# L-Scofano/SEEME

Measured on AMD Instinct MI355X. Metric: sampled seqs/sec (T=196, 50 DDIM steps), higher is better.
Workload: dtype f32 accumulate (fp16 denoiser weights, fp16 VAE MFMA operands); 1 GPU; config_mld_egobody interactee-only: VAE encode -> 50-step DDIM -> VAE decode, B=32/GPU, T=196, nfeats=132, random-init recipe weights; batch_per_gpu=32, seq_len=196, ddim_steps=50, parallelism=dp1 (independent shards, no collective on the data path)

## Files before the change

include/seeme_hip.h:

```cpp
#ifndef SEEME_HIP_H
#define SEEME_HIP_H

#include <stddef.h>
#include <stdint.h>

#ifdef __cplusplus
extern "C" {
#endif

#define SEEME_D 256
#define SEEME_NLAYERS 5

enum { SEEME_ACT_NONE = 0, SEEME_ACT_RELU = 1, SEEME_ACT_GELU = 2, SEEME_ACT_SILU = 3 };
enum { SEEME_SCHED_NONE = 0, SEEME_SCHED_DDIM = 1, SEEME_SCHED_DDPM = 2 };

int seeme_version(void);
const char* seeme_last_error(void);

#define SEEME_LINEAR_MAX_K 1008
typedef struct {
    const float* A;  int lda;
    const float* A2; int lda2;
    int K1;
    const float* W;  int ldw;
// ... 11 lines not shown

typedef struct {
    const float *in_w, *in_b;
    const float *out_w, *out_b;
    const float *l1_w, *l1_b;
    const float *l2_w, *l2_b;
    const float *n1_w, *n1_b, *n2_w, *n2_b;
    const float *ca_in_w, *ca_in_b;
    const float *ca_out_w, *ca_out_b;
    const float *n3_w, *n3_b;
} SeemeXfLayer;

typedef struct {
    SeemeXfLayer layer[SEEME_NLAYERS];
    const float *skip_w[2], *skip_b[2];
    const float *norm_w, *norm_b;
} SeemeSkipStack;

typedef struct { const uint16_t *in_w, *out_w, *l1_w, *l2_w; } SeemeXfLayerH;
typedef struct {
    SeemeXfLayerH enc[SEEME_NLAYERS], dec[SEEME_NLAYERS];
    const uint16_t *enc_skip[2], *dec_skip[2];
    const uint16_t *emb_w, *fin_w, *ca_fold_w;
    const void* dec_pro; int dec_pro_T;
} SeemeVaeWeightsH;

typedef struct {
    int nfeats;
    int ff;
    const float* token;
    const float* pe_enc;
    const float* pe_dec;
    const float* emb_w; int emb_ldw;
    const float* emb_b;
    const float* fin_w;
    const float* fin_b;
    SeemeSkipStack enc, dec;
    const float* ca_fold_w;
    const float* ca_fold_b;
    const SeemeVaeWeightsH* h16;
} SeemeVaeWeights;

size_t seeme_vae_workspace_bytes(int B, int T);

int seeme_vae_encode(const SeemeVaeWeights* w, const float* features, const int32_t* lengths,
                     int B, int T, float* mu, float* logvar, void* workspace, size_t ws_bytes, void* stream);

// ... 430 lines not shown
```

seeme_amd/_lib.py:

```python
from __future__ import annotations

import ctypes as C
import os
from typing import Optional

_HERE = os.path.dirname(os.path.abspath(__file__))
LIB_PATH = os.environ.get("SEEME_HIP_LIB") or os.path.join(_HERE, "libseeme_hip.so")

NLAYERS = 5
TROW = 7680
CROW = 5120
ACT_NONE, ACT_RELU, ACT_GELU, ACT_SILU = 0, 1, 2, 3
SCHED_NONE, SCHED_DDIM, SCHED_DDPM = 0, 1, 2

fp = C.c_void_p


class SeemeError(RuntimeError):
    pass


class LinearArgs(C.Structure):
    _fields_ = [("A", fp), ("lda", C.c_int), ("A2", fp), ("lda2", C.c_int), ("K1", C.c_int),
                ("W", fp), ("ldw", C.c_int), ("bias", fp), ("res", fp), ("ldr", C.c_int),
                ("ln_w", fp), ("ln_b", fp), ("pre_ln_w", fp), ("pre_ln_b", fp),
                ("Y", fp), ("ldy", C.c_int), ("M", C.c_int), ("N", C.c_int), ("K", C.c_int),
                ("pre_act", C.c_int), ("act", C.c_int), ("eps", C.c_float)]


class XfLayer(C.Structure):
    _fields_ = [(n, fp) for n in ("in_w", "in_b", "out_w", "out_b", "l1_w", "l1_b", "l2_w", "l2_b",
                                  "n1_w", "n1_b", "n2_w", "n2_b",
                                  "ca_in_w", "ca_in_b", "ca_out_w", "ca_out_b", "n3_w", "n3_b")]


class SkipStack(C.Structure):
    _fields_ = [("layer", XfLayer * NLAYERS), ("skip_w", fp * 2), ("skip_b", fp * 2),
                ("norm_w", fp), ("norm_b", fp)]


class XfLayerH(C.Structure):
    _fields_ = [(n, fp) for n in ("in_w", "out_w", "l1_w", "l2_w")]


class VaeWeightsH(C.Structure):
    _fields_ = [("enc", XfLayerH * NLAYERS), ("dec", XfLayerH * NLAYERS), ("enc_skip", fp * 2), ("dec_skip", fp * 2),
                ("emb_w", fp), ("fin_w", fp), ("ca_fold_w", fp), ("dec_pro", fp), ("dec_pro_T", C.c_int)]


def pack_mfma16(W, dtype):
    import torch
    N, K = W.shape
    Np, Kp = (N + 15) // 16 * 16, (K + 31) // 32 * 32
    Wz = torch.zeros(Np, Kp, device=W.device, dtype=dtype)
    Wz[:N, :K] = W.detach().to(dtype)
    return Wz.view(Np // 16, 16, Kp // 32, 4, 8).permute(0, 2, 3, 1, 4).contiguous()


class VaeWeights(C.Structure):
    _fields_ = [("nfeats", C.c_int), ("ff", C.c_int), ("token", fp), ("pe_enc", fp), ("pe_dec", fp),
                ("emb_w", fp), ("emb_ldw", C.c_int), ("emb_b", fp), ("fin_w", fp), ("fin_b", fp),
                ("enc", SkipStack), ("dec", SkipStack), ("ca_fold_w", fp), ("ca_fold_b", fp), ("h16", fp)]


class DenoiserWeights(C.Structure):
    _fields_ = [("wg", fp), ("wdtype", C.c_int), ("vp", fp), ("layout", fp), ("nhead", C.c_int), ("ff_sa", C.c_int),
                ("ff", C.c_int), ("kv_cat_w", fp), ("kv_cat_b", fp), ("style_cat_w", fp), ("style_cat_b", fp),
                ("time_w1", fp), ("time_b1", fp), ("time_w2", fp), ("time_b2", fp),
                ("ca_kv_w", fp * NLAYERS), ("ca_kv_b", fp * NLAYERS),
                ("ca_tn_w", fp * NLAYERS), ("ca_tn_b", fp * NLAYERS),
# ... 285 lines not shown
```

seeme_amd/csrc/vae_h16.hip:

```cpp
#include "common.hpp"
#include "api_util.hpp"

typedef _Float16 h16x8 __attribute__((ext_vector_type(8)));
#define HPAD 16

__device__ __forceinline__ unsigned short f2h(float x) { return __builtin_bit_cast(unsigned short, (_Float16)x); }
__device__ __forceinline__ float h_exp(float x) { return __builtin_amdgcn_exp2f(x * 1.44269504088896340736f); }
__device__ __forceinline__ float h_gelu(float x) {
    const float z = fabsf(x) * 0.70710678118654752440f;
    const float t = __builtin_amdgcn_rcpf(fmaf(0.3275911f, z, 1.f));
    const float poly = t * fmaf(t, fmaf(t, fmaf(t, fmaf(t, 1.061405429f, -1.453152027f), 1.421413741f), -0.284496736f), 0.254829592f);
    return 0.5f * x * (1.f + copysignf(1.f - poly * h_exp(-z * z), x));
}
__device__ __forceinline__ float h_act(float v, int act) { return act == SEEME_ACT_GELU ? h_gelu(v) : act_apply(v, act); }

#ifdef H16_DBG_TIMES
__device__ unsigned long long h16_dbg_times[32];
#ifndef H16_DBG_KERNEL
#define H16_DBG_KERNEL 1
#endif
#define H16_DBG(k, i) do { if (H16_DBG_KERNEL == (k) && blockIdx.x == 3 && blockIdx.y == ((k) == 1 ? 5 : 0) && threadIdx.x == 0) h16_dbg_times[i] = __builtin_readcyclecounter(); } while (0)
extern "C" int seeme_debug_h16_times(unsigned long long* host, int n) {
    SEEME_HIP(hipMemcpyFromSymbol(host, HIP_SYMBOL(h16_dbg_times), sizeof(unsigned long long) * (size_t)(n < 32 ? n : 32)));
    return 0;
// ... 691 lines not shown
#ifndef LAYER_KV_PF
#define LAYER_KV_PF 4
#endif
#ifndef LAYER_W8_PF
#define LAYER_W8_PF 4
#endif
#ifndef LAYER_WPE
#define LAYER_WPE 2
#endif
struct LayerHArgs {
    const unsigned short* q; const uint4* kp; const uint4* vp; const float* res;
    const uint4* wo; const float* bo; const float* n1_w; const float* n1_b;
    const int32_t* lengths;
    int S, n_prefix, q_rows, Sp, spv; float scale, eps;
    const float* cvec; int cvec_ld; const float* lnc_w; const float* lnc_b;
    const uint4* w1; const float* b1; const uint4* w2; const float* b2; const float* n2_w; const float* n2_b;
    const float* fin_w; const float* fin_b;
    float* out; int out_mode, B;
    int in_shared;
    const uint4* skip_w; const float* skip_b; const float* skip_src; float* xnext;
    const uint4* qkv_w; const float* qkv_b; unsigned short* q_out; uint4* kp_out; uint4* vp_out;
    const uint4* proj_w; const float* proj_b; float* feats; int F;
    const float* z; const uint4* cf_w; const float* cf_b; int layer;
};
template <int WAVES, int RW>
__host__ __device__ constexpr bool layer_cvec_in() { return WAVES == 8 && RW == 4; }

__device__ __forceinline__ void rows_to_h16(unsigned short* Xh, int ldh, int row, int lane, float4 v) {
    const unsigned lo = (unsigned)f2h(v.x) | ((unsigned)f2h(v.y) << 16), hi = (unsigned)f2h(v.z) | ((unsigned)f2h(v.w) << 16);
    *reinterpret_cast<uint2*>(Xh + row * ldh + lane * 4) = make_uint2(lo, hi);
}

template <int WAVES, int RW>
__device__ __forceinline__ void tail_store_q(const unsigned short* Oh, int ld, unsigned short* __restrict__ q_out, size_t base, int q0, int S) {
    constexpr int NT = 64 * WAVES;
    const int tid = threadIdx.x;
#pragma unroll
    for (int it = 0; it < RW / 2; ++it) {
        const int idx = tid + it * NT, row = idx >> 5, c8 = (idx & 31) * 8, s = q0 + row;
        if (s < S) *reinterpret_cast<uint4*>(q_out + (base + s) * 256 + c8) = *reinterpret_cast<const uint4*>(Oh + row * ld + c8);
    }
}
template <int WAVES, int RW>
__device__ __forceinline__ void tail_store_k(const unsigned short* Oh, int ld, uint4* __restrict__ kp_out, int b, int q0, int S, int NT16) {
    constexpr int NT = 64 * WAVES;
    const int tid = threadIdx.x;
// ... 48 lines not shown
    {
        f32x4 acc[MTL][NTL];
        acc_zero(acc);
        const BiasRegs<NTL> bias = bias_load<NTL>(qkv_b, 1 * 256 + wave * CW, 768);
        gemm_packed<MTL, NTL, PF>(Xh, ldq, qkv_w, 8, 1 * 16 + wave * NTL, 48, 8, acc, ring_t);
        prime_packed(ring_t, qkv_w, 8, 2 * 16 + wave * NTL, 48, 8);
        acc_store_h16<MTL, NTL>(acc, OhK, ldk, wave * CW, bias, SEEME_ACT_NONE);
    }
    {
        f32x4 acc[MTL][NTL];
        acc_zero(acc);
        const BiasRegs<NTL> bias = bias_load<NTL>(qkv_b, 2 * 256 + wave * CW, 768);
        gemm_packed<MTL, NTL, PF>(Xh, ldq, qkv_w, 8, 2 * 16 + wave * NTL, 48, 8, acc, ring_t);
        __syncthreads();
        tail_store_q<WAVES, RW>(Oh, ldq, q_out, base, q0, S);
        tail_store_k<WAVES, RW>(OhK, ldk, kp_out, b, q0, S, NT16);
        __syncthreads();
        acc_store_h16<MTL, NTL>(acc, Oh, ldq, wave * CW, bias, SEEME_ACT_NONE);
        __syncthreads();
        tail_store_v<WAVES, RW>(Oh, ldq, vp_out, b, q0, S, KB);
    }
}

#define LAYER_DBG(i) do { if (a.qkv_w != nullptr) H16_DBG(5, i); } while (0)
template <int WAVES, int RW>
__global__ __launch_bounds__(64 * WAVES, WAVES == 4 ? LAYER_WPE : 1) void k_layer_h(const LayerHArgs a) {
    constexpr int ROWS = RW * WAVES, MTL = ROWS / 16, NTL = 16 / WAVES, CW = 256 / WAVES, N1 = 8 / WAVES, NT = 64 * WAVES;
    constexpr int PFW = (WAVES == 8 && RW == 4) ? LAYER_W8_PF : H16_PF, PFA = (WAVES == 8 && RW == 4) ? LAYER_W8_PF : ATT_PF,
                  PFK = (WAVES == 8 && RW == 4) ? LAYER_W8_PF : LAYER_KV_PF, PFF = (WAVES == 8 && RW == 4) ? LAYER_W8_PF : FFN_PF;
    extern __shared__ __attribute__((aligned(16))) float smem[];
    const int tid = threadIdx.x, wave = tid >> 6, lane = tid & 63, r = lane & 15, kq = lane >> 4;
    const int ldp = a.Sp + LDS_PAD, ldq = 256 + HPAD, ldph = 2 * ldp, ldc = 256 + LDS_PAD;
    float* R0 = smem;
    unsigned short* R1 = reinterpret_cast<unsigned short*>(R0 + ROWS * ldp);
    float* Ps = R0;
    unsigned short* Ph = reinterpret_cast<unsigned short*>(R0);
    unsigned short* Qh = R1;
    int b = blockIdx.y, qt = blockIdx.x;
    if ((gridDim.y & 7) == 0) {
        const int L = blockIdx.x + gridDim.x * blockIdx.y, rr = L & 7, q = L >> 3;
        b = rr + 8 * (q / (int)gridDim.x);
        qt = q % (int)gridDim.x;
    }
    const int q0 = qt * ROWS;
    const size_t base = (size_t)b * a.S;
    const size_t bin = a.in_shared ? 0 : (size_t)b, base_in = bin * a.S;
    const int n_valid_keys = min(a.S, a.n_prefix + a.lengths[b]);
    const BiasRegs<NTL> bias_o = bias_load<NTL>(a.bo, wave * CW, 256);
    BRing<NTL, PFA> ring_o;
    prime_packed(ring_o, a.wo, 8, wave * NTL, 16, 8);
    const bool cv_in = layer_cvec_in<WAVES, RW>() && a.z != nullptr;
    unsigned short* Zh = R1 + ROWS * ldq;
    float* CVs = reinterpret_cast<float*>(Zh + 16 * ldq);
    const int cv_t0 = 16 * a.layer + wave * NTL;
    BRing<NTL, 8> ring_c;
    BiasRegs<NTL> bias_c;
    if (cv_in) {
        bias_c = bias_load<NTL>(a.cf_b + 256 * a.layer, wave * CW, 256);
        for (int i = tid; i < 15 * ldq / 8; i += NT) reinterpret_cast<uint4*>(Zh + ldq)[i] = make_uint4(0u, 0u, 0u, 0u);
        if (wave == 0) rows_to_h16(Zh, ldq, 0, lane, *reinterpret_cast<const float4*>(a.z + (size_t)b * 256 + lane * 4));
    }
    LAYER_DBG(0);
    {
        uint4 qv[4];
#pragma unroll
        for (int it = 0; it < RW / 2; ++it) {
            const int idx = tid + it * NT, row = idx >> 5, c8 = (idx & 31) * 8, s = q0 + row;
            qv[it] = *reinterpret_cast<const uint4*>(a.q + (base_in + (s < a.q_rows ? s : 0)) * 256 + c8);
            if (s >= a.q_rows) qv[it] = make_uint4(0u, 0u, 0u, 0u);
        }
#pragma unroll
        for (int it = 0; it < RW / 2; ++it) {
            const int idx = tid + it * NT, row = idx >> 5, c8 = (idx & 31) * 8;
            *reinterpret_cast<uint4*>(Qh + row * ldq + c8) = qv[it];
        }
    }
    __syncthreads();
    LAYER_DBG(1);
    const int NT16 = (a.S + 15) >> 4;
    const uint4* Kp = a.kp + bin * NT16 * 512;
    for (int c0 = 0; c0 < a.Sp; c0 += CH_N) {
        const int n0 = c0 + wave * CW;
        f32x4 acc[MTL][NTL];
        acc_zero(acc);
        if (n0 < a.S) gemm_packed<MTL, NTL, PFK>(Qh, ldq, Kp, 8, n0 >> 4, NT16, 8, acc);
#pragma unroll
        for (int nt = 0; nt < NTL; ++nt) {
            const int c = n0 + nt * 16 + r;
            const bool ok = c < n_valid_keys;
#pragma unroll
            for (int mt = 0; mt < MTL; ++mt)
#pragma unroll
                for (int i = 0; i < 4; ++i) Ps[(mt * 16 + 4 * kq + i) * ldp + c] = ok ? acc[mt][nt][i] * a.scale : -INFINITY;
        }
    }
    __syncthreads();
    LAYER_DBG(2);
    if (cv_in) prime_packed(ring_c, a.cf_w, 8, cv_t0, 16 * SEEME_NLAYERS, 8);
    LAYER_DBG(21);
    if (a.Sp == 256) attn_softmax_rows<4, RW>(Ps, ldp, Ph, ldph, wave, lane);
    else attn_softmax_rows<8, RW>(Ps, ldp, Ph, ldph, wave, lane);
    __syncthreads();
    LAYER_DBG(3);
    if (cv_in) {
        f32x4 acc_c[1][NTL];
        acc_zero(acc_c);
        gemm_packed<1, NTL, 8>(Zh, ldq, a.cf_w, 8, cv_t0, 16 * SEEME_NLAYERS, 8, acc_c, ring_c);
        if (kq == 0) {
#pragma unroll
            for (int nt = 0; nt < NTL; ++nt) CVs[wave * CW + nt * 16 + r] = acc_c[0][nt][0] + bias_c.v[nt];
        }
    }
    LAYER_DBG(22);
    {
        f32x4 acc[MTL][NTL];
        acc_zero(acc);
        const int K32 = (n_valid_keys + 31) >> 5;
        gemm_packed<MTL, NTL, PFK>(Ph, ldph, a.vp + bin * 16 * (a.spv >> 5) * 64, a.spv >> 5, wave * NTL, 16, K32, acc);
        acc_store_h16<MTL, NTL>(acc, Qh, ldq, wave * CW, nullptr, SEEME_ACT_NONE);
    }
    __syncthreads();
    LAYER_DBG(4);
    float* Cs = R0;
    {
        f32x4 acc[MTL][NTL];
        acc_zero(acc);
        gemm_packed<MTL, NTL, PFA>(Qh, ldq, a.wo, 8, wave * NTL, 16, 8, acc, ring_o);
#ifdef H16_DBG_TIMES
        asm volatile("" : "+v"(acc[0][0][0]), "+v"(acc[MTL - 1][NTL - 1][3]));
        LAYER_DBG(23);
#endif
        acc_store_lds<MTL, NTL>(acc, Cs, ldc, wave * CW, bias_o, SEEME_ACT_NONE);
    }
    LAYER_DBG(24);
    const BiasRegs<N1> bias1 = bias_load<N1>(a.b1, wave * (128 / WAVES), 128);
    const BiasRegs<NTL> bias2 = bias_load<NTL>(a.b2, wave * CW, 256);
    BRing<N1, PFF> ring1;
    BRing<NTL, PFW> ring2;
    prime_packed(ring1, a.w1, 8, wave * N1, 8, 8);
    prime_packed(ring2, a.w2, 4, wave * NTL, 16, 4);
    LAYER_DBG(25);
    __syncthreads();
    LAYER_DBG(5);
    unsigned short* Xh = R1;
    float4 x1[RW];
    {
        const LnParams lp = ln_params256_opt(a.n1_w, a.n1_b, a.n1_w), lc = ln_params256_opt(a.lnc_w, a.lnc_b, a.n1_w);
        float4 xr[RW];
        const bool has_cv = cv_in || a.cvec != nullptr;
        const float4 cv = cv_in ? *reinterpret_cast<const float4*>(CVs + lane * 4)
                                : *reinterpret_cast<const float4*>((a.cvec != nullptr ? a.cvec + (size_t)b * a.cvec_ld : a.n1_w) + lane * 4);
#pragma unroll
        for (int rr = 0; rr < RW; ++rr) {
            const int s = q0 + wave * RW + rr;
            xr[rr] = *reinterpret_cast<const float4*>(a.res + (base_in + (s < a.q_rows ? s : 0)) * 256 + lane * 4);
        }
        __builtin_amdgcn_sched_barrier(0);
        LAYER_DBG(16);
#pragma unroll
        for (int rr = 0; rr < RW; ++rr) {
            const float4 v = *reinterpret_cast<const float4*>(Cs + (wave * RW + rr) * ldc + lane * 4);
            x1[rr] = make_float4(v.x + xr[rr].x, v.y + xr[rr].y, v.z + xr[rr].z, v.w + xr[rr].w);
        }
        LAYER_DBG(17);
        wave_layernorm256_rows<RW>(x1, lp, a.eps);
        LAYER_DBG(18);
        if (has_cv) {
#pragma unroll
            for (int rr = 0; rr < RW; ++rr) x1[rr] = make_float4(x1[rr].x + cv.x, x1[rr].y + cv.y, x1[rr].z + cv.z, x1[rr].w + cv.w);
            wave_layernorm256_rows<RW>(x1, lc, a.eps);
        }
        LAYER_DBG(19);
#pragma unroll
        for (int rr = 0; rr < RW; ++rr) {
            const int row = wave * RW + rr;
            if (q0 + row >= a.q_rows) x1[rr] = make_float4(0.f, 0.f, 0.f, 0.f);
            rows_to_h16(Xh, ldq, row, lane, x1[rr]);
        }
        LAYER_DBG(20);
    }
    __syncthreads();
    LAYER_DBG(6);
    unsigned short* Hh = R1;
    const int ldhh = 128 + HPAD;
    {
        f32x4 acc1[MTL][N1];
        acc_zero(acc1);
        gemm_packed<MTL, N1, PFF>(Xh, ldq, a.w1, 8, wave * N1, 8, 8, acc1, ring1);
        __syncthreads();
// ... 72 lines not shown
        __syncthreads();
    }
    LAYER_DBG(10);
    if (a.qkv_w != nullptr) {
        tail_qkv_rows<WAVES, RW, PFW>(Xh, reinterpret_cast<unsigned short*>(R0), a.qkv_w, a.qkv_b, a.q_out, a.kp_out, a.vp_out, b, q0, a.S, a.spv, ring_t);
        LAYER_DBG(11);
        return;
    }
    if (a.proj_w != nullptr) {
        const int ntiles = (a.F + 15) >> 4;
        const BiasRegs<NTL> bias = bias_load<NTL>(a.proj_b, wave * CW, a.F);
        f32x4 acc[MTL][NTL];
        acc_zero(acc);
        if (wave * NTL < ntiles) gemm_packed<MTL, NTL, PFW>(Xh, ldq, a.proj_w, 8, wave * NTL, ntiles, 8, acc, ring_t);
        acc_store_lds<MTL, NTL>(acc, Cs, ldc, wave * CW, bias, SEEME_ACT_NONE);
        __syncthreads();
        for (int idx = tid; idx < ROWS * 256; idx += NT) {
            const int row = idx >> 8, c = idx & 255, s = q0 + row;
            if (s < a.S && c < a.F) a.feats[(base + s) * a.F + c] = Cs[row * ldc + c];
        }
    }
}

template <int WAVES, int RW>
static int launch_layer_w(const LayerHArgs& a, hipStream_t st) {
    constexpr int ROWS = RW * WAVES;
    if (a.z != nullptr && !layer_cvec_in<WAVES, RW>()) return seeme_fail("layer_h: this instantiation does not form the cross-attention vector");
    const size_t lds = (size_t)ROWS * (a.Sp + LDS_PAD) * 4 + (size_t)ROWS * (256 + HPAD) * 2 +
                       (layer_cvec_in<WAVES, RW>() ? (size_t)16 * (256 + HPAD) * 2 + 256 * 4 : 0);
    dim3 grid((a.q_rows + ROWS - 1) / ROWS, a.B);
    SEEME_HIP(hipFuncSetAttribute((const void*)k_layer_h<WAVES, RW>, hipFuncAttributeMaxDynamicSharedMemorySize, (int)lds));
    hipLaunchKernelGGL((k_layer_h<WAVES, RW>), grid, dim3(64 * WAVES), lds, st, a);
    return seeme_check_launch("k_layer_h");
}
static int layer_form(int B, int q_rows, int S) {
    static int rows = -1, w8_max = -1;
    if (rows < 0) { const char* e = getenv("SEEME_LAYER_ROWS"); rows = e ? atoi(e) : 32; }
    if (w8_max < 0) { const char* e = getenv("SEEME_LAYER_W8_MAX"); w8_max = e ? atoi(e) : 256; }
    const int Sp = (S + CH_N - 1) / CH_N * CH_N;
    if (rows == 64 && Sp <= 256 && q_rows > 32) return 2;
    const long wgs = (long)B * ((q_rows + 31) / 32);
    return wgs <= w8_max ? 1 : 0;
}
static bool layer_forms_cvec(int B, int q_rows, int S) { return layer_form(B, q_rows, S) == 1; }
static int launch_layer_h(const LayerHArgs& a_in, hipStream_t st) {
    LayerHArgs a = a_in;
    if (a.S <= 0 || a.S > 512) return seeme_fail("layer_h: S must be in 1..512");
    a.Sp = (a.S + CH_N - 1) / CH_N * CH_N;
    const int form = layer_form(a.B, a.q_rows, a.S);
    if (form == 2) return launch_layer_w<8, 8>(a, st);
    return form == 1 ? launch_layer_w<8, 4>(a, st) : launch_layer_w<4, 8>(a, st);
}


struct ProHArgs {
    int mode, B, S, T, F, spv;
    const float* features; const uint4* emb_w; const float* emb_b; const float* token; const float* pe;
    float* x;
    const uint4* qkv_w; const float* qkv_b; unsigned short* q_out; uint4* kp_out; uint4* vp_out;
};
template <int NB, bool VEC>
__device__ __forceinline__ void pro_stage_features(const ProHArgs& a, unsigned short* __restrict__ R1, int lda_h, int b, int q0, int tid) {
    const unsigned bytes = (unsigned)a.T * (unsigned)a.F * 4u;
    const __amdgpu_buffer_rsrc_t rs = __builtin_amdgcn_make_buffer_rsrc(const_cast<float*>(a.features + (size_t)b * a.T * a.F), 0, (int)bytes, 0x00020000);
    if (VEC) {
        const int row = tid >> 3, sl = tid & 7, s = q0 + row;
        const bool rok = s >= 2 && s < a.S;
        const unsigned ro = (unsigned)(s - 2) * (unsigned)a.F * 4u;
        float4 v[NB];
#pragma unroll
        for (int j = 0; j < NB; ++j) {
            const int c = 4 * (sl + 8 * j);
            const bool ok = rok && (j < NB - 1 || c < a.F);
// ... 258 lines not shown
        ProHArgs p{};
        p.mode = 1; p.B = B; p.S = S; p.T = T; p.F = F; p.spv = ws.spv; p.features = features; p.emb_w = (const uint4*)H->emb_w;
        p.emb_b = w->emb_b; p.token = w->token; p.pe = w->pe_enc; p.x = ws.x;
        p.qkv_w = (const uint4*)H->enc[0].in_w; p.qkv_b = E.layer[0].in_b; p.q_out = kv[0].q; p.kp_out = kv[0].kp; p.vp_out = kv[0].vp;
        if ((rc = launch_pro_h(p, st))) return rc;
    }
    LayerHArgs a = layer_args(E.layer[0], H->enc[0], kv[0], ws.x, lengths, B, S, ws.spv, 2, S, nullptr, 0);
    a.out = ws.sk0; tail_qkv(a, E.layer[1], H->enc[1], kv[1]);
    if ((rc = launch_layer_h(a, st))) return rc;
    a = layer_args(E.layer[1], H->enc[1], kv[1], ws.sk0, lengths, B, S, ws.spv, 2, S, nullptr, 0);
    a.out = ws.sk1; tail_qkv(a, E.layer[2], H->enc[2], kv[0]);
    if ((rc = launch_layer_h(a, st))) return rc;
    a = layer_args(E.layer[2], H->enc[2], kv[0], ws.sk1, lengths, B, S, ws.spv, 2, S, nullptr, 0);
    tail_skip(a, H->enc_skip[0], E.skip_b[0], ws.sk1, ws.x); tail_qkv(a, E.layer[3], H->enc[3], kv[1]);
    if ((rc = launch_layer_h(a, st))) return rc;
    a = layer_args(E.layer[3], H->enc[3], kv[1], ws.x, lengths, B, S, ws.spv, 2, S, nullptr, 0);
    tail_skip(a, H->enc_skip[1], E.skip_b[1], ws.sk0, ws.x); tail_qkv(a, E.layer[4], H->enc[4], kv[0]);
    if ((rc = launch_layer_h(a, st))) return rc;
    a = layer_args(E.layer[4], H->enc[4], kv[0], ws.x, lengths, B, S, ws.spv, 2, 2, nullptr, 0);
    a.out = mu; a.out_mode = 1; a.fin_w = E.norm_w; a.fin_b = E.norm_b;
    return launch_layer_h(a, st);
}

struct DecPro { float* x; KvSet kv; };
static DecPro carve_dec_pro(void* buf, int T) {
    char* p = static_cast<char*>(buf);
    DecPro d;
    d.x = reinterpret_cast<float*>(p); p += (size_t)T * 256 * 4;
    d.kv.q = reinterpret_cast<unsigned short*>(p); p += (size_t)T * 256 * 2;
    d.kv.kp = reinterpret_cast<uint4*>(p); p += (size_t)((T + 15) >> 4) * 512 * 16;
    d.kv.vp = reinterpret_cast<uint4*>(p);
    return d;
}
extern "C" size_t seeme_vae_dec_prologue_bytes(int T) {
    if (T < 1) return 0;
    return (size_t)T * 256 * 6 + (size_t)((T + 15) >> 4) * 512 * 16 + (size_t)((T + 31) >> 5) * 16 * 64 * 16;
}
static int launch_dec_pro(const SeemeVaeWeights* w, int T, float* x, const KvSet& kv, hipStream_t st) {
    ProHArgs p{};
    p.mode = 2; p.B = 1; p.S = T; p.T = T; p.F = w->nfeats; p.spv = (T + 31) & ~31; p.pe = w->pe_dec; p.x = x;
    p.qkv_w = (const uint4*)w->h16->dec[0].in_w; p.qkv_b = w->dec.layer[0].in_b; p.q_out = kv.q; p.kp_out = kv.kp; p.vp_out = kv.vp;
    return launch_pro_h(p, st);
}
extern "C" int seeme_vae_dec_prologue_h16(const SeemeVaeWeights* w, int T, void* buf, size_t bytes, void* stream) {
    if (w == nullptr || w->h16 == nullptr) return seeme_fail("vae_dec_prologue: fp16 weight image missing");
    if (T < 1 || T > 512) return seeme_fail("vae_dec_prologue: T must be in 1..512");
    if (buf == nullptr || (reinterpret_cast<size_t>(buf) & 15) != 0) return seeme_fail("vae_dec_prologue: buffer must be 16-byte aligned");
    if (bytes < seeme_vae_dec_prologue_bytes(T)) return seeme_fail("vae_dec_prologue: buffer too small");
    const DecPro d = carve_dec_pro(buf, T);
    return launch_dec_pro(w, T, d.x, d.kv, (hipStream_t)stream);
}

int seeme_vae_decode_h16(const SeemeVaeWeights* w, const float* z, const int32_t* lengths, int B, int T, float* feats,
                         void* workspace, hipStream_t st) {
    const SeemeVaeWeightsH* H = w->h16;
    const int S = T, F = w->nfeats;
    WsH ws = carve_h(workspace, B, S + 2);
    ws.spv = (S + 31) & ~31;
    if (!vae_fused_enabled() || ws.spv > 2 * S || F > 256) return vae_decode_h16_unfused(w, z, lengths, B, T, feats, workspace, st);
    const SeemeSkipStack& Dk = w->dec;
    KvSet kv[2];
    kv_sets(ws, B, kv);
    int rc;
    const int CL = SEEME_NLAYERS * 256;
    const bool cv_in = layer_forms_cvec(B, S, S);
    if (!cv_in && (rc = lin_h(st, z, 256, H->ca_fold_w, 256, CL, w->ca_fold_b, ws.cvec, CL, B))) return rc;
    auto dec_args = [&](int l, const KvSet& in, const float* res) {
        LayerHArgs a = layer_args(Dk.layer[l], H->dec[l], in, res, lengths, B, S, ws.spv, 0, S, ws.cvec + l * 256, CL);
        if (cv_in) { a.cvec = nullptr; a.z = z; a.cf_w = (const uint4*)H->ca_fold_w; a.cf_b = w->ca_fold_b; a.layer = l; }
        return a;
    };
    KvSet in0 = kv[0];
    const float* res0 = ws.x;
    if (H->dec_pro != nullptr && H->dec_pro_T == T) {
        const DecPro d = carve_dec_pro(const_cast<void*>(H->dec_pro), T);
        in0 = d.kv; res0 = d.x;
    } else if ((rc = launch_dec_pro(w, T, ws.x, kv[0], st))) return rc;
    LayerHArgs a = dec_args(0, in0, res0);
    a.in_shared = 1;
    a.out = ws.sk0; tail_qkv(a, Dk.layer[1], H->dec[1], kv[1]);
    if ((rc = launch_layer_h(a, st))) return rc;
    a = dec_args(1, kv[1], ws.sk0);
    a.out = ws.sk1; tail_qkv(a, Dk.layer[2], H->dec[2], kv[0]);
    if ((rc = launch_layer_h(a, st))) return rc;
    a = dec_args(2, kv[0], ws.sk1);
    tail_skip(a, H->dec_skip[0], Dk.skip_b[0], ws.sk1, ws.x); tail_qkv(a, Dk.layer[3], H->dec[3], kv[1]);
    if ((rc = launch_layer_h(a, st))) return rc;
    a = dec_args(3, kv[1], ws.x);
    tail_skip(a, H->dec_skip[1], Dk.skip_b[1], ws.sk0, ws.x); tail_qkv(a, Dk.layer[4], H->dec[4], kv[0]);
    if ((rc = launch_layer_h(a, st))) return rc;
    a = dec_args(4, kv[0], ws.x);
    a.fin_w = Dk.norm_w; a.fin_b = Dk.norm_b; a.proj_w = (const uint4*)H->fin_w; a.proj_b = w->fin_b; a.feats = feats; a.F = F;
    return launch_layer_h(a, st);
}
```

seeme_amd/mld_vae.py:

```python
from __future__ import annotations

import ctypes as C
from typing import List, Optional

import torch
import torch.nn as nn

from . import _lib as L


class _PositionEmbeddingLearned1D(nn.Module):

    def __init__(self, d_model: int, max_len: int = 500):
        super().__init__()
        self.pe = nn.Parameter(torch.zeros(max_len, 1, d_model))
        nn.init.uniform_(self.pe)


class _EncoderLayerParams(nn.Module):

    def __init__(self, d_model, nhead, ff, dropout):
        super().__init__()
        self.d_model = d_model
        self.self_attn = nn.MultiheadAttention(d_model, nhead, dropout=dropout)
        self.linear1 = nn.Linear(d_model, ff)
# ... 76 lines not shown
        if position_embedding not in ("v3", "learned"):
            raise NotImplementedError("only the learned 1D position embedding is on the accelerated path")
        if self.arch != "encoder_decoder":
            if self.arch == "all_encoder":
                raise NotImplementedError("arch 'all_encoder' is outside the accelerated path (motion_vae.yaml uses encoder_decoder)")
            raise ValueError("Not support architecture!")
        if self.mlp_dist:
            raise NotImplementedError("MLP_DIST=True is outside the accelerated path")
        if normalize_before or activation != "gelu" or self.latent_dim != 256 or self.latent_size != 1:
            raise NotImplementedError("accelerated path: post-norm, gelu, latent_dim [1,256]")

        d = self.latent_dim
        self.query_pos_encoder = _PositionEmbeddingLearned1D(d)
        self.query_pos_decoder = _PositionEmbeddingLearned1D(d)
        self.encoder = _SkipStackParams(lambda: _EncoderLayerParams(d, num_heads, ff_size, dropout), num_layers, d)
        self.decoder = _SkipStackParams(lambda: _DecoderLayerParams(d, num_heads, ff_size, dropout), num_layers, d)
        self.global_motion_token = nn.Parameter(torch.randn(self.latent_size * 2, d))
        self.skel_embedding = nn.Linear(nfeats, d)
        self.final_layer = nn.Linear(d, nfeats)

        self._wcache = None
        self._ws = L.Workspace(per_stream=False)
        self._dec_pro = {}

    dec_prologue_cache = True
    _DEC_PRO_MAX = 8

    def _weights(self) -> L.VaeWeights:
        fpnt = (_param_fingerprint(self), self.precision)
        if self._wcache is not None and self._wcache[0] == fpnt:
            return self._wcache[1]
        for p in self.parameters():
            L.require_cuda(p, "MldVae parameter")
            if not p.is_contiguous():
                raise L.SeemeError("MldVae parameters must be contiguous")
        keep = []
        w = L.VaeWeights()
        w.nfeats, w.ff = self.nfeats, self.ff_size
        w.token = L.ptr(self.global_motion_token)
        w.pe_enc = L.ptr(self.query_pos_encoder.pe)
        w.pe_dec = L.ptr(self.query_pos_decoder.pe)
        F = self.nfeats
        Fp = (F + 15) // 16 * 16
        with torch.no_grad():
            embw = torch.zeros(self.latent_dim, Fp, device=self.skel_embedding.weight.device, dtype=torch.float32)
            embw[:, :F] = self.skel_embedding.weight
# ... 31 lines not shown
        w.h16 = 0
        h = None
        if self.precision == "fp16":
            h = L.VaeWeightsH()
            pk = lambda W: (keep.append(L.pack_mfma16(W, torch.float16)), keep[-1].data_ptr())[1]
            for stack, dst in ((self.encoder, h.enc), (self.decoder, h.dec)):
                for i, blk in enumerate(stack.blocks()):
                    dst[i].in_w, dst[i].out_w = pk(blk.self_attn.in_proj_weight), pk(blk.self_attn.out_proj.weight)
                    dst[i].l1_w, dst[i].l2_w = pk(blk.linear1.weight), pk(blk.linear2.weight)
            for i in range(2):
                h.enc_skip[i] = pk(self.encoder.linear_blocks[i].weight)
                h.dec_skip[i] = pk(self.decoder.linear_blocks[i].weight)
            h.emb_w, h.fin_w, h.ca_fold_w = pk(self.skel_embedding.weight), pk(self.final_layer.weight), pk(fold_w)
            keep.append(h)
            w.h16 = C.addressof(h)
        self._wcache = (fpnt, w, keep, h)
        self._dec_pro = {}
        return w

    def _dec_prologue(self, w: L.VaeWeights, T: int, device) -> None:
        h = self._wcache[3]
        if h is None:
            return
        h.dec_pro, h.dec_pro_T = 0, 0
        if not self.dec_prologue_cache:
            return
        buf = self._dec_pro.get(T)
        if buf is None:
            if torch.cuda.is_current_stream_capturing():
                return
            if len(self._dec_pro) >= self._DEC_PRO_MAX:
                self._dec_pro.clear()
            need = L.lib().seeme_vae_dec_prologue_bytes(T)
            buf = torch.zeros(need, dtype=torch.uint8, device=device)
            L.call("seeme_vae_dec_prologue_h16", C.byref(w), T, buf.data_ptr(), buf.numel(), L.current_stream())
            torch.cuda.current_stream().synchronize()
            self._dec_pro[T] = buf
        h.dec_pro, h.dec_pro_T = buf.data_ptr(), T

    def _workspace(self, B: int, T: int, device) -> torch.Tensor:
        return self._ws.get(L.lib().seeme_vae_workspace_bytes(B, T), device)

    @staticmethod
    def _lengths_tensor(lengths, device) -> torch.Tensor:
        key = (tuple(int(v) for v in lengths), str(device))
        t = MldVae._LEN_CACHE.get(key)
        if t is None:
            if len(MldVae._LEN_CACHE) > 64:
                MldVae._LEN_CACHE.clear()
            t = torch.as_tensor(list(key[0]), dtype=torch.int32).to(device)
            MldVae._LEN_CACHE[key] = t
        return t

    _LEN_CACHE: dict = {}

    def forward(self, features, lengths: Optional[List[int]] = None):
        z, dist = self.encode(features, None, lengths)
        return self.decode(z, lengths), z, dist

    def encode_dist(self, features: torch.Tensor, lengths: Optional[List[int]] = None) -> torch.Tensor:
        L.require_cuda(features, "features")
# ... 44 lines not shown
```

Baseline: 17860 seqs/s.

## Cache decoder layer-0 post-attention rows in prologue and skip attention for full-length batches

```diff
diff --git a/include/seeme_hip.h b/include/seeme_hip.h
--- a/include/seeme_hip.h
+++ b/include/seeme_hip.h
@@ -57,7 +57,7 @@
     SeemeXfLayerH enc[SEEME_NLAYERS], dec[SEEME_NLAYERS];
     const uint16_t *enc_skip[2], *dec_skip[2];
     const uint16_t *emb_w, *fin_w, *ca_fold_w;
-    const void* dec_pro; int dec_pro_T;
+    const void* dec_pro; int dec_pro_T; int dec_l0;
 } SeemeVaeWeightsH;
 
 typedef struct {
diff --git a/seeme_amd/_lib.py b/seeme_amd/_lib.py
--- a/seeme_amd/_lib.py
+++ b/seeme_amd/_lib.py
@@ -45,7 +45,7 @@
 
 class VaeWeightsH(C.Structure):
     _fields_ = [("enc", XfLayerH * NLAYERS), ("dec", XfLayerH * NLAYERS), ("enc_skip", fp * 2), ("dec_skip", fp * 2),
-                ("emb_w", fp), ("fin_w", fp), ("ca_fold_w", fp), ("dec_pro", fp), ("dec_pro_T", C.c_int)]
+                ("emb_w", fp), ("fin_w", fp), ("ca_fold_w", fp), ("dec_pro", fp), ("dec_pro_T", C.c_int), ("dec_l0", C.c_int)]
 
 
 def pack_mfma16(W, dtype):
diff --git a/seeme_amd/csrc/vae_h16.hip b/seeme_amd/csrc/vae_h16.hip
--- a/seeme_amd/csrc/vae_h16.hip
+++ b/seeme_amd/csrc/vae_h16.hip
@@ -737,6 +737,7 @@
     const uint4* qkv_w; const float* qkv_b; unsigned short* q_out; uint4* kp_out; uint4* vp_out;
     const uint4* proj_w; const float* proj_b; float* feats; int F;
     const float* z; const uint4* cf_w; const float* cf_b; int layer;
+    const float* x1_in; float* x1_out;
 };
 template <int WAVES, int RW>
 __host__ __device__ constexpr bool layer_cvec_in() { return WAVES == 8 && RW == 4; }
@@ -831,9 +832,14 @@
     }
 }
 
+#ifdef H16_DBG_L0
+#define LAYER_DBG(i) do { if (a.in_shared != 0 && a.x1_out == nullptr) H16_DBG(5, i); } while (0)
+#else
 #define LAYER_DBG(i) do { if (a.qkv_w != nullptr) H16_DBG(5, i); } while (0)
-template <int WAVES, int RW>
+#endif
+template <int WAVES, int RW, bool L0 = false>
 __global__ __launch_bounds__(64 * WAVES, WAVES == 4 ? LAYER_WPE : 1) void k_layer_h(const LayerHArgs a) {
+    static_assert(!L0 || layer_cvec_in<WAVES, RW>(), "the entry past the attention block needs the vector formed in the layer");
     constexpr int ROWS = RW * WAVES, MTL = ROWS / 16, NTL = 16 / WAVES, CW = 256 / WAVES, N1 = 8 / WAVES, NT = 64 * WAVES;
     constexpr int PFW = (WAVES == 8 && RW == 4) ? LAYER_W8_PF : H16_PF, PFA = (WAVES == 8 && RW == 4) ? LAYER_W8_PF : ATT_PF,
                   PFK = (WAVES == 8 && RW == 4) ? LAYER_W8_PF : LAYER_KV_PF, PFF = (WAVES == 8 && RW == 4) ? LAYER_W8_PF : FFN_PF;
@@ -854,64 +860,14 @@
     const int q0 = qt * ROWS;
     const size_t base = (size_t)b * a.S;
     const size_t bin = a.in_shared ? 0 : (size_t)b, base_in = bin * a.S;
-    const int n_valid_keys = min(a.S, a.n_prefix + a.lengths[b]);
-    const BiasRegs<NTL> bias_o = bias_load<NTL>(a.bo, wave * CW, 256);
-    BRing<NTL, PFA> ring_o;
-    prime_packed(ring_o, a.wo, 8, wave * NTL, 16, 8);
+    const bool l0_build = L0 && a.x1_out != nullptr;
     const bool cv_in = layer_cvec_in<WAVES, RW>() && a.z != nullptr;
     unsigned short* Zh = R1 + ROWS * ldq;
     float* CVs = reinterpret_cast<float*>(Zh + 16 * ldq);
     const int cv_t0 = 16 * a.layer + wave * NTL;
     BRing<NTL, 8> ring_c;
     BiasRegs<NTL> bias_c;
-    if (cv_in) {
-        bias_c = bias_load<NTL>(a.cf_b + 256 * a.layer, wave * CW, 256);
-        for (int i = tid; i < 15 * ldq / 8; i += NT) reinterpret_cast<uint4*>(Zh + ldq)[i] = make_uint4(0u, 0u, 0u, 0u);
-        if (wave == 0) rows_to_h16(Zh, ldq, 0, lane, *reinterpret_cast<const float4*>(a.z + (size_t)b * 256 + lane * 4));
-    }
-    LAYER_DBG(0);
-    {
-        uint4 qv[4];
-#pragma unroll
-        for (int it = 0; it < RW / 2; ++it) {
-            const int idx = tid + it * NT, row = idx >> 5, c8 = (idx & 31) * 8, s = q0 + row;
-            qv[it] = *reinterpret_cast<const uint4*>(a.q + (base_in + (s < a.q_rows ? s : 0)) * 256 + c8);
-            if (s >= a.q_rows) qv[it] = make_uint4(0u, 0u, 0u, 0u);
-        }
-#pragma unroll
-        for (int it = 0; it < RW / 2; ++it) {
-            const int idx = tid + it * NT, row = idx >> 5, c8 = (idx & 31) * 8;
-            *reinterpret_cast<uint4*>(Qh + row * ldq + c8) = qv[it];
-        }
-    }
-    __syncthreads();
-    LAYER_DBG(1);
-    const int NT16 = (a.S + 15) >> 4;
-    const uint4* Kp = a.kp + bin * NT16 * 512;
-    for (int c0 = 0; c0 < a.Sp; c0 += CH_N) {
-        const int n0 = c0 + wave * CW;
-        f32x4 acc[MTL][NTL];
-        acc_zero(acc);
-        if (n0 < a.S) gemm_packed<MTL, NTL, PFK>(Qh, ldq, Kp, 8, n0 >> 4, NT16, 8, acc);
-#pragma unroll
-        for (int nt = 0; nt < NTL; ++nt) {
-            const int c = n0 + nt * 16 + r;
-            const bool ok = c < n_valid_keys;
-#pragma unroll
-            for (int mt = 0; mt < MTL; ++mt)
-#pragma unroll
-                for (int i = 0; i < 4; ++i) Ps[(mt * 16 + 4 * kq + i) * ldp + c] = ok ? acc[mt][nt][i] * a.scale : -INFINITY;
-        }
-    }
-    __syncthreads();
-    LAYER_DBG(2);
-    if (cv_in) prime_packed(ring_c, a.cf_w, 8, cv_t0, 16 * SEEME_NLAYERS, 8);
-    LAYER_DBG(21);
-    if (a.Sp == 256) attn_softmax_rows<4, RW>(Ps, ldp, Ph, ldph, wave, lane);
-    else attn_softmax_rows<8, RW>(Ps, ldp, Ph, ldph, wave, lane);
-    __syncthreads();
-    LAYER_DBG(3);
-    if (cv_in) {
+    auto form_cvec = [&]() {
         f32x4 acc_c[1][NTL];
         acc_zero(acc_c);
         gemm_packed<1, NTL, 8>(Zh, ldq, a.cf_w, 8, cv_t0, 16 * SEEME_NLAYERS, 8, acc_c, ring_c);
@@ -919,61 +875,167 @@
 #pragma unroll
             for (int nt = 0; nt < NTL; ++nt) CVs[wave * CW + nt * 16 + r] = acc_c[0][nt][0] + bias_c.v[nt];
         }
-    }
-    LAYER_DBG(22);
-    {
-        f32x4 acc[MTL][NTL];
-        acc_zero(acc);
-        const int K32 = (n_valid_keys + 31) >> 5;
-        gemm_packed<MTL, NTL, PFK>(Ph, ldph, a.vp + bin * 16 * (a.spv >> 5) * 64, a.spv >> 5, wave * NTL, 16, K32, acc);
-        acc_store_h16<MTL, NTL>(acc, Qh, ldq, wave * CW, nullptr, SEEME_ACT_NONE);
-    }
-    __syncthreads();
-    LAYER_DBG(4);
+    };
+    const bool l0_skip = L0 && cv_in && a.x1_in != nullptr && a.n_prefix + a.lengths[b] >= a.S;
+    unsigned short* Xh = R1;
     float* Cs = R0;
-    {
-        f32x4 acc[MTL][NTL];
-        acc_zero(acc);
-        gemm_packed<MTL, NTL, PFA>(Qh, ldq, a.wo, 8, wave * NTL, 16, 8, acc, ring_o);
-#ifdef H16_DBG_TIMES
-        asm volatile("" : "+v"(acc[0][0][0]), "+v"(acc[MTL - 1][NTL - 1][3]));
-        LAYER_DBG(23);
-#endif
-        acc_store_lds<MTL, NTL>(acc, Cs, ldc, wave * CW, bias_o, SEEME_ACT_NONE);
-    }
-    LAYER_DBG(24);
-    const BiasRegs<N1> bias1 = bias_load<N1>(a.b1, wave * (128 / WAVES), 128);
-    const BiasRegs<NTL> bias2 = bias_load<NTL>(a.b2, wave * CW, 256);
+    float4 x1[RW], cv;
+    LnParams lc;
+    bool has_cv;
+    BiasRegs<N1> bias1;
+    BiasRegs<NTL> bias2;
     BRing<N1, PFF> ring1;
     BRing<NTL, PFW> ring2;
-    prime_packed(ring1, a.w1, 8, wave * N1, 8, 8);
-    prime_packed(ring2, a.w2, 4, wave * NTL, 16, 4);
-    LAYER_DBG(25);
-    __syncthreads();
-    LAYER_DBG(5);
-    unsigned short* Xh = R1;
-    float4 x1[RW];
-    {
-        const LnParams lp = ln_params256_opt(a.n1_w, a.n1_b, a.n1_w), lc = ln_params256_opt(a.lnc_w, a.lnc_b, a.n1_w);
-        float4 xr[RW];
-        const bool has_cv = cv_in || a.cvec != nullptr;
-        const float4 cv = cv_in ? *reinterpret_cast<const float4*>(CVs + lane * 4)
-                                : *reinterpret_cast<const float4*>((a.cvec != nullptr ? a.cvec + (size_t)b * a.cvec_ld : a.n1_w) + lane * 4);
+    if (l0_skip) {
+        lc = ln_params256_opt(a.lnc_w, a.lnc_b, a.n1_w);
 #pragma unroll
         for (int rr = 0; rr < RW; ++rr) {
             const int s = q0 + wave * RW + rr;
-            xr[rr] = *reinterpret_cast<const float4*>(a.res + (base_in + (s < a.q_rows ? s : 0)) * 256 + lane * 4);
-        }
+            x1[rr] = *reinterpret_cast<const float4*>(a.x1_in + (size_t)(s < a.q_rows ? s : 0) * 256 + lane * 4);
+        }
+        const float4 zv = *reinterpret_cast<const float4*>(a.z + (size_t)b * 256 + lane * 4);
+        bias_c = bias_load<NTL>(a.cf_b + 256 * a.layer, wave * CW, 256);
         __builtin_amdgcn_sched_barrier(0);
+        LAYER_DBG(0);
+        prime_packed(ring_c, a.cf_w, 8, cv_t0, 16 * SEEME_NLAYERS, 8);
+        bias1 = bias_load<N1>(a.b1, wave * (128 / WAVES), 128);
+        bias2 = bias_load<NTL>(a.b2, wave * CW, 256);
+        prime_packed(ring1, a.w1, 8, wave * N1, 8, 8);
+        prime_packed(ring2, a.w2, 4, wave * NTL, 16, 4);
+        __builtin_amdgcn_sched_barrier(0);
+        LAYER_DBG(1);
+        LAYER_DBG(2);
+        LAYER_DBG(21);
+        for (int i = tid; i < 15 * ldq / 8; i += NT) reinterpret_cast<uint4*>(Zh + ldq)[i] = make_uint4(0u, 0u, 0u, 0u);
+        if (wave == 0) rows_to_h16(Zh, ldq, 0, lane, zv);
+        __syncthreads();
+        LAYER_DBG(3);
+        form_cvec();
+        LAYER_DBG(22);
+        LAYER_DBG(4);
+        LAYER_DBG(23);
+        LAYER_DBG(24);
+        LAYER_DBG(25);
+        __syncthreads();
+        LAYER_DBG(5);
         LAYER_DBG(16);
-#pragma unroll
-        for (int rr = 0; rr < RW; ++rr) {
-            const float4 v = *reinterpret_cast<const float4*>(Cs + (wave * RW + rr) * ldc + lane * 4);
-            x1[rr] = make_float4(v.x + xr[rr].x, v.y + xr[rr].y, v.z + xr[rr].z, v.w + xr[rr].w);
-        }
+        cv = *reinterpret_cast<const float4*>(CVs + lane * 4);
+        has_cv = true;
         LAYER_DBG(17);
-        wave_layernorm256_rows<RW>(x1, lp, a.eps);
-        LAYER_DBG(18);
+    } else {
+        const int n_valid_keys = min(a.S, a.n_prefix + a.lengths[b]);
+        const BiasRegs<NTL> bias_o = bias_load<NTL>(a.bo, wave * CW, 256);
+        BRing<NTL, PFA> ring_o;
+        prime_packed(ring_o, a.wo, 8, wave * NTL, 16, 8);
+        if (cv_in) {
+            bias_c = bias_load<NTL>(a.cf_b + 256 * a.layer, wave * CW, 256);
+            for (int i = tid; i < 15 * ldq / 8; i += NT) reinterpret_cast<uint4*>(Zh + ldq)[i] = make_uint4(0u, 0u, 0u, 0u);
+            if (wave == 0) rows_to_h16(Zh, ldq, 0, lane, *reinterpret_cast<const float4*>(a.z + (size_t)b * 256 + lane * 4));
+        }
+        LAYER_DBG(0);
+        {
+            uint4 qv[4];
+#pragma unroll
+            for (int it = 0; it < RW / 2; ++it) {
+                const int idx = tid + it * NT, row = idx >> 5, c8 = (idx & 31) * 8, s = q0 + row;
+                qv[it] = *reinterpret_cast<const uint4*>(a.q + (base_in + (s < a.q_rows ? s : 0)) * 256 + c8);
+                if (s >= a.q_rows) qv[it] = make_uint4(0u, 0u, 0u, 0u);
+            }
+#pragma unroll
+            for (int it = 0; it < RW / 2; ++it) {
+                const int idx = tid + it * NT, row = idx >> 5, c8 = (idx & 31) * 8;
+                *reinterpret_cast<uint4*>(Qh + row * ldq + c8) = qv[it];
+            }
+        }
+        __syncthreads();
+        LAYER_DBG(1);
+        const int NT16 = (a.S + 15) >> 4;
+        const uint4* Kp = a.kp + bin * NT16 * 512;
+        for (int c0 = 0; c0 < a.Sp; c0 += CH_N) {
+            const int n0 = c0 + wave * CW;
+            f32x4 acc[MTL][NTL];
+            acc_zero(acc);
+            if (n0 < a.S) gemm_packed<MTL, NTL, PFK>(Qh, ldq, Kp, 8, n0 >> 4, NT16, 8, acc);
+#pragma unroll
+            for (int nt = 0; nt < NTL; ++nt) {
+                const int c = n0 + nt * 16 + r;
+                const bool ok = c < n_valid_keys;
+#pragma unroll
+                for (int mt = 0; mt < MTL; ++mt)
+#pragma unroll
+                    for (int i = 0; i < 4; ++i) Ps[(mt * 16 + 4 * kq + i) * ldp + c] = ok ? acc[mt][nt][i] * a.scale : -INFINITY;
+            }
+        }
+        __syncthreads();
+        LAYER_DBG(2);
+        if (cv_in) prime_packed(ring_c, a.cf_w, 8, cv_t0, 16 * SEEME_NLAYERS, 8);
+        LAYER_DBG(21);
+        if (a.Sp == 256) attn_softmax_rows<4, RW>(Ps, ldp, Ph, ldph, wave, lane);
+        else attn_softmax_rows<8, RW>(Ps, ldp, Ph, ldph, wave, lane);
+        __syncthreads();
+        LAYER_DBG(3);
+        if (cv_in) form_cvec();
+        LAYER_DBG(22);
+        {
+            f32x4 acc[MTL][NTL];
+            acc_zero(acc);
+            const int K32 = (n_valid_keys + 31) >> 5;
+            gemm_packed<MTL, NTL, PFK>(Ph, ldph, a.vp + bin * 16 * (a.spv >> 5) * 64, a.spv >> 5, wave * NTL, 16, K32, acc);
+            acc_store_h16<MTL, NTL>(acc, Qh, ldq, wave * CW, nullptr, SEEME_ACT_NONE);
+        }
+        __syncthreads();
+        LAYER_DBG(4);
+        {
+            f32x4 acc[MTL][NTL];
+            acc_zero(acc);
+            gemm_packed<MTL, NTL, PFA>(Qh, ldq, a.wo, 8, wave * NTL, 16, 8, acc, ring_o);
+#ifdef H16_DBG_TIMES
+            asm volatile("" : "+v"(acc[0][0][0]), "+v"(acc[MTL - 1][NTL - 1][3]));
+            LAYER_DBG(23);
+#endif
+            acc_store_lds<MTL, NTL>(acc, Cs, ldc, wave * CW, bias_o, SEEME_ACT_NONE);
+        }
+        LAYER_DBG(24);
+        bias1 = bias_load<N1>(a.b1, wave * (128 / WAVES), 128);
+        bias2 = bias_load<NTL>(a.b2, wave * CW, 256);
+        prime_packed(ring1, a.w1, 8, wave * N1, 8, 8);
+        prime_packed(ring2, a.w2, 4, wave * NTL, 16, 4);
+        LAYER_DBG(25);
+        __syncthreads();
+        LAYER_DBG(5);
+        {
+            const LnParams lp = ln_params256_opt(a.n1_w, a.n1_b, a.n1_w);
+            lc = ln_params256_opt(a.lnc_w, a.lnc_b, a.n1_w);
+            float4 xr[RW];
+            has_cv = cv_in || a.cvec != nullptr;
+            cv = cv_in ? *reinterpret_cast<const float4*>(CVs + lane * 4)
+                       : *reinterpret_cast<const float4*>((a.cvec != nullptr ? a.cvec + (size_t)b * a.cvec_ld : a.n1_w) + lane * 4);
+#pragma unroll
+            for (int rr = 0; rr < RW; ++rr) {
+                const int s = q0 + wave * RW + rr;
+                xr[rr] = *reinterpret_cast<const float4*>(a.res + (base_in + (s < a.q_rows ? s : 0)) * 256 + lane * 4);
+            }
+            __builtin_amdgcn_sched_barrier(0);
+            LAYER_DBG(16);
+#pragma unroll
+            for (int rr = 0; rr < RW; ++rr) {
+                const float4 v = *reinterpret_cast<const float4*>(Cs + (wave * RW + rr) * ldc + lane * 4);
+                x1[rr] = make_float4(v.x + xr[rr].x, v.y + xr[rr].y, v.z + xr[rr].z, v.w + xr[rr].w);
+            }
+            LAYER_DBG(17);
+            wave_layernorm256_rows<RW>(x1, lp, a.eps);
+        }
+        if (l0_build) {
+#pragma unroll
+            for (int rr = 0; rr < RW; ++rr) {
+                const int s = q0 + wave * RW + rr;
+                if (s < a.q_rows) *reinterpret_cast<float4*>(a.x1_out + (size_t)s * 256 + lane * 4) = x1[rr];
+            }
+            return;
+        }
+    }
+    LAYER_DBG(18);
+    {
         if (has_cv) {
 #pragma unroll
             for (int rr = 0; rr < RW; ++rr) x1[rr] = make_float4(x1[rr].x + cv.x, x1[rr].y + cv.y, x1[rr].z + cv.z, x1[rr].w + cv.w);
@@ -1092,15 +1154,16 @@
     }
 }
 
-template <int WAVES, int RW>
+template <int WAVES, int RW, bool L0 = false>
 static int launch_layer_w(const LayerHArgs& a, hipStream_t st) {
     constexpr int ROWS = RW * WAVES;
     if (a.z != nullptr && !layer_cvec_in<WAVES, RW>()) return seeme_fail("layer_h: this instantiation does not form the cross-attention vector");
+    if ((a.x1_in != nullptr || a.x1_out != nullptr) != L0) return seeme_fail("layer_h: rows after norm1 passed to the wrong instantiation");
     const size_t lds = (size_t)ROWS * (a.Sp + LDS_PAD) * 4 + (size_t)ROWS * (256 + HPAD) * 2 +
                        (layer_cvec_in<WAVES, RW>() ? (size_t)16 * (256 + HPAD) * 2 + 256 * 4 : 0);
     dim3 grid((a.q_rows + ROWS - 1) / ROWS, a.B);
-    SEEME_HIP(hipFuncSetAttribute((const void*)k_layer_h<WAVES, RW>, hipFuncAttributeMaxDynamicSharedMemorySize, (int)lds));
-    hipLaunchKernelGGL((k_layer_h<WAVES, RW>), grid, dim3(64 * WAVES), lds, st, a);
+    SEEME_HIP(hipFuncSetAttribute((const void*)k_layer_h<WAVES, RW, L0>, hipFuncAttributeMaxDynamicSharedMemorySize, (int)lds));
+    hipLaunchKernelGGL((k_layer_h<WAVES, RW, L0>), grid, dim3(64 * WAVES), lds, st, a);
     return seeme_check_launch("k_layer_h");
 }
 static int layer_form(int B, int q_rows, int S) {
@@ -1119,6 +1182,8 @@
     a.Sp = (a.S + CH_N - 1) / CH_N * CH_N;
     const int form = layer_form(a.B, a.q_rows, a.S);
     if (form == 2) return launch_layer_w<8, 8>(a, st);
+    if (form != 1) a.x1_in = nullptr;
+    if (form == 1 && a.x1_in != nullptr) return launch_layer_w<8, 4, true>(a, st);
     return form == 1 ? launch_layer_w<8, 4>(a, st) : launch_layer_w<4, 8>(a, st);
 }
 
@@ -1423,19 +1488,22 @@
     return launch_layer_h(a, st);
 }
 
-struct DecPro { float* x; KvSet kv; };
+static bool dec_fused(int T, int F) { return vae_fused_enabled() && ((T + 31) & ~31) <= 2 * T && F <= 256; }
+struct DecPro { float* x; KvSet kv; float* x1; int32_t* len; };
 static DecPro carve_dec_pro(void* buf, int T) {
     char* p = static_cast<char*>(buf);
     DecPro d;
     d.x = reinterpret_cast<float*>(p); p += (size_t)T * 256 * 4;
     d.kv.q = reinterpret_cast<unsigned short*>(p); p += (size_t)T * 256 * 2;
     d.kv.kp = reinterpret_cast<uint4*>(p); p += (size_t)((T + 15) >> 4) * 512 * 16;
-    d.kv.vp = reinterpret_cast<uint4*>(p);
+    d.kv.vp = reinterpret_cast<uint4*>(p); p += (size_t)((T + 31) >> 5) * 16 * 64 * 16;
+    d.x1 = reinterpret_cast<float*>(p); p += (size_t)T * 256 * 4;
+    d.len = reinterpret_cast<int32_t*>(p);
     return d;
 }
 extern "C" size_t seeme_vae_dec_prologue_bytes(int T) {
     if (T < 1) return 0;
-    return (size_t)T * 256 * 6 + (size_t)((T + 15) >> 4) * 512 * 16 + (size_t)((T + 31) >> 5) * 16 * 64 * 16;
+    return (size_t)T * 256 * 10 + (size_t)((T + 15) >> 4) * 512 * 16 + (size_t)((T + 31) >> 5) * 16 * 64 * 16 + 16;
 }
 static int launch_dec_pro(const SeemeVaeWeights* w, int T, float* x, const KvSet& kv, hipStream_t st) {
     ProHArgs p{};
@@ -1449,7 +1517,14 @@
     if (buf == nullptr || (reinterpret_cast<size_t>(buf) & 15) != 0) return seeme_fail("vae_dec_prologue: buffer must be 16-byte aligned");
     if (bytes < seeme_vae_dec_prologue_bytes(T)) return seeme_fail("vae_dec_prologue: buffer too small");
     const DecPro d = carve_dec_pro(buf, T);
-    return launch_dec_pro(w, T, d.x, d.kv, (hipStream_t)stream);
+    int rc;
+    if ((rc = launch_dec_pro(w, T, d.x, d.kv, (hipStream_t)stream))) return rc;
+    if (!dec_fused(T, w->nfeats)) return 0;
+    SEEME_HIP(hipMemsetD32Async(reinterpret_cast<hipDeviceptr_t>(d.len), T, 1, (hipStream_t)stream));
+    LayerHArgs a = layer_args(w->dec.layer[0], w->h16->dec[0], d.kv, d.x, d.len, 1, T, (T + 31) & ~31, 0, T, nullptr, 0);
+    a.in_shared = 1; a.x1_out = d.x1;
+    a.Sp = (T + CH_N - 1) / CH_N * CH_N;
+    return launch_layer_w<8, 4, true>(a, (hipStream_t)stream);
 }
 
 int seeme_vae_decode_h16(const SeemeVaeWeights* w, const float* z, const int32_t* lengths, int B, int T, float* feats,
@@ -1458,7 +1533,7 @@
     const int S = T, F = w->nfeats;
     WsH ws = carve_h(workspace, B, S + 2);
     ws.spv = (S + 31) & ~31;
-    if (!vae_fused_enabled() || ws.spv > 2 * S || F > 256) return vae_decode_h16_unfused(w, z, lengths, B, T, feats, workspace, st);
+    if (!dec_fused(T, F)) return vae_decode_h16_unfused(w, z, lengths, B, T, feats, workspace, st);
     const SeemeSkipStack& Dk = w->dec;
     KvSet kv[2];
     kv_sets(ws, B, kv);
@@ -1473,12 +1548,14 @@
     };
     KvSet in0 = kv[0];
     const float* res0 = ws.x;
+    const float* x1_0 = nullptr;
     if (H->dec_pro != nullptr && H->dec_pro_T == T) {
         const DecPro d = carve_dec_pro(const_cast<void*>(H->dec_pro), T);
         in0 = d.kv; res0 = d.x;
+        if (H->dec_l0 && cv_in) x1_0 = d.x1;
     } else if ((rc = launch_dec_pro(w, T, ws.x, kv[0], st))) return rc;
     LayerHArgs a = dec_args(0, in0, res0);
-    a.in_shared = 1;
+    a.in_shared = 1; a.x1_in = x1_0;
     a.out = ws.sk0; tail_qkv(a, Dk.layer[1], H->dec[1], kv[1]);
     if ((rc = launch_layer_h(a, st))) return rc;
     a = dec_args(1, kv[1], ws.sk0);
diff --git a/seeme_amd/mld_vae.py b/seeme_amd/mld_vae.py
--- a/seeme_amd/mld_vae.py
+++ b/seeme_amd/mld_vae.py
@@ -1,6 +1,7 @@
 from __future__ import annotations
 
 import ctypes as C
+import os
 from typing import List, Optional
 
 import torch
@@ -123,6 +124,7 @@
         self._wcache = None
         self._ws = L.Workspace(per_stream=False)
         self._dec_pro = {}
+        self.dec_layer0 = os.environ.get("SEEME_VAE_DEC_L0", "1") != "0"
 
     dec_prologue_cache = True
     _DEC_PRO_MAX = 8
@@ -200,7 +202,7 @@
         h = self._wcache[3]
         if h is None:
             return
-        h.dec_pro, h.dec_pro_T = 0, 0
+        h.dec_pro, h.dec_pro_T, h.dec_l0 = 0, 0, 0
         if not self.dec_prologue_cache:
             return
         buf = self._dec_pro.get(T)
@@ -214,7 +216,7 @@
             L.call("seeme_vae_dec_prologue_h16", C.byref(w), T, buf.data_ptr(), buf.numel(), L.current_stream())
             torch.cuda.current_stream().synchronize()
             self._dec_pro[T] = buf
-        h.dec_pro, h.dec_pro_T = buf.data_ptr(), T
+        h.dec_pro, h.dec_pro_T, h.dec_l0 = buf.data_ptr(), T, int(self.dec_layer0)
 
     def _workspace(self, B: int, T: int, device) -> torch.Tensor:
         return self._ws.get(L.lib().seeme_vae_workspace_bytes(B, T), device)
```

Result: no change. 17900 seqs/s, median of 6 (+0.2%).
